# EPFL-IMOS/simple-SFOD

Hardware: AMD Instinct MI355X
Metric: teacher+student train images/s on 1024x2048 synthetic (higher is better)
Workload: dtype bf16x3

## Files before the change

### include/sfod_hip.h

```cpp
#ifndef SFOD_HIP_H
#define SFOD_HIP_H
#include <stdint.h>
#ifdef __cplusplus
extern "C" {
#endif

#define SFOD_F32 0
#define SFOD_BF16 1
#define SFOD_BF16X3 2
#define SFOD_F16X3 3

int sfod_version(void);
const char* sfod_last_error(void);

int sfod_preprocess(const void* const* img_ptrs, const int32_t* sizes, int B, int Hp, int Wp,
                    int Cpad, const float* mean3, const float* std3, void* out, int dt,
                    void* stream);

int sfod_hflip_u8(const void* src, void* dst, int C, int H, int W, void* stream);

int sfod_resize_bilinear_u8(const void* src, void* dst, int C, int H, int W, int h, int w,
                            const int32_t* hbounds, const int32_t* hcoef, int ksize_h,
                            const int32_t* vbounds, const int32_t* vcoef, int ksize_v, int flip,
                            void* stream);

int sfod_conv_fwd(const void* x, const void* w, const float* bias, void* y, int B, int H, int W,
                  int Cin, int Cout, int ksize, int ldy, int act, float* stats, int dt, int out_dt,
                  void* stream);
int sfod_conv_fwd_ws(const void* x, const void* w, const uint32_t* w_absmax, const float* bias, void* y, int B, int H,
                     int W, int Cin, int Cout, int ksize, int ldy, int act, float* stats, int dt, int out_dt,
                     void* stream);
int64_t sfod_conv_fwd_scratch_bytes(int B, int H, int W, int Cin, int Cout, int ksize, int dt, int out_dt, int with_stats);
int sfod_conv_fwd_scratch(const void* x, const void* w, const uint32_t* w_absmax, const float* bias, void* y, int B, int H,
                          int W, int Cin, int Cout, int ksize, int ldy, int act, float* stats, int dt, int out_dt,
                          void* scratch, int64_t scratch_bytes, void* stream);
int sfod_conv_stats_blocks(int B, int H, int W, int Cin, int Cout, int ksize, int dt);
int sfod_set_conv_algo(int algo);
int sfod_conv_dgrad_bnred_blocks(int B, int H, int W, int Cin, int Cout, int dt);
int sfod_conv_dgrad_bnred(const void* x, const void* w, void* dz, int B, int H, int W, int Cin, int Cout, int dt,
                          const float* y, const float* mean, const float* invstd, const float* gamma,
                          const float* beta, float* red_ws, void* stream);
int sfod_conv_fwd_bnin_supported(int B, int H, int W, int Cin, int Cout, int dt);
int sfod_conv_fwd_bnin(const float* x_pre, const float* in_mean, const float* in_invstd, const float* in_gamma,
                       const float* in_beta, const void* w, const float* bias, float* y, int B, int H, int W, int Cin,
                       int Cout, int ldy, int act, float* stats, int dt, void* stream);
int sfod_set_gemm_tile(int tile);
int sfod_set_conv3x3_variant(int variant);
int sfod_last_conv_kernel(char* buf, int n);
int sfod_set_deterministic(int on);
int sfod_get_deterministic(void);
int sfod_set_conv3x3_m16(int on);
int sfod_set_wgrad3x3_pipe(int on);
int sfod_conv_fwd_algo(int B, int H, int W, int Cin, int Cout, int ksize, int dt);

int sfod_conv_first_supported(int B, int H, int W, int Cin, int Cout, int dt, int ldy);
int sfod_conv_first_fused(const void* x, const void* w, const float* bias, const float* scale,
                          const float* shift, void* y, float* stats, int B, int H, int W, int ldy,
                          int act, int dt, void* stream);
int sfod_conv_first_fused_ws(const void* x, const void* w, const uint32_t* w_absmax, const float* bias,
                             const float* scale, const float* shift, void* y, float* stats, int B, int H, int W,
                             int ldy, int act, int dt, void* stream);

int64_t sfod_conv_wgrad_ws_bytes(int B, int H, int W, int Cin, int Cout, int ksize, int lddy, int dt);
int sfod_conv_wgrad(const void* x, const void* dy, float* dw, int B, int H, int W, int Cin,
                    int Cout, int ksize, int lddy, int dt, void* ws, int64_t ws_bytes, void* stream);
int sfod_conv_wgrad_oihw_supported(int B, int H, int W, int Cin, int Cout, int ksize, int lddy, int dt);
int sfod_conv_wgrad_oihw(const void* x, const void* dy, float* dw_oihw, int B, int H, int W, int Cin,
                         int Cout, int ksize, int lddy, int dt, int accumulate, void* ws,
                         int64_t ws_bytes, void* stream);

int sfod_pack_conv_weight(const float* w_oihw, void* w_packed, int Cout, int Cin, int ksize,
                          int CinPad, int rot180, int dt, void* stream);
int sfod_pack_conv_weight_ws(const float* w_oihw, void* w_packed, uint32_t* absmax, int Cout, int Cin, int ksize,
                             int CinPad, int rot180, int dt, void* stream);
int sfod_pack_conv_weights_blocks(int Cout, int Cin, int ksize, int innerPad, int rot180);
int sfod_pack_conv_weights_multi(const int64_t* desc, int n, int total_blocks, int dt, void* stream);
int sfod_pack_conv_weights_multi_ws(const int64_t* desc, int n, int total_blocks, int dt, uint32_t* absmax ,
                                    void* stream);
int sfod_unpack_conv_wgrad(const float* dw_packed, float* dw_oihw, int Cout, int Cin, int ksize,
                           int CinPad, int accumulate, void* stream);
int sfod_pack_fc_weight(const float* w, void* out, int N, int K, int chw_c, int transpose, int dt,
                        void* stream);
int sfod_unpack_fc_wgrad(const float* dw_packed, float* dw, int N, int K, int chw_c,
                         int accumulate, void* stream);
int sfod_pack_fc_weight_ld(const float* w, void* out, int N, int K, int chw_c, int transpose, int ld,
                           int dt, void* stream);
int sfod_pack_fc_weight_ld_ws(const float* w, void* out, uint32_t* absmax, int N, int K, int chw_c, int transpose,
                              int ld, int dt, void* stream);
int sfod_unpack_fc_wgrad_ld(const float* dw_packed, float* dw, int N, int K, int chw_c, int ld,
                            int accumulate, void* stream);
int sfod_bias_grad(const void* dy, float* db, int M, int N, int ld, int accumulate, int dt,
                   void* stream);

int sfod_bn_finalize(const float* stats, int nblocks, int M, int C,
                     float* mean, float* invstd, float* running_mean, float* running_var,
                     float momentum, float eps, int update_running, int64_t* num_batches_tracked,
                     float* ws, void* stream);
int sfod_set_bn_finalize_fused(int on);
int sfod_bn_finalize_ws_floats(int C);
int sfod_bn_relu_pool_fwd(const void* y, const float* mean, const float* invstd,
                          const float* gamma, const float* beta, void* z, int B, int H, int W,
                          int C, int pool, int dt, int out_dt, void* stream);
int sfod_bn_relu_pool_fwd2(const void* y, const float* mean, const float* invstd,
                           const float* gamma, const float* beta, void* z, void* z2, int B, int H, int W,
                           int C, int pool, int dt, int out_dt, void* stream);
int sfod_bn_add_relu_fwd(const void* y, const float* mean, const float* invstd, const float* gamma,
                         const float* beta, const void* residual, void* z, void* z_pairs, void* z_pairs2, int64_t rows,
                         int C, int dt, int pairs_dt, void* stream);
int sfod_bn_relu_pool_bwd(const void* dz, const void* y, const float* mean, const float* invstd,
                          const float* gamma, const float* beta, void* dy, float* dgamma,
                          float* dbeta, float* dgamma_acc, float* dbeta_acc, float* ws, int B, int H,
                          int W, int C, int pool, int dt, int out_dt, int reduced_blocks, void* stream);
#define SFOD_BN_BWD_SCRATCH_ROWS 32
int sfod_bn_bwd_ws_floats(int M, int C);
int sfod_add_act(const void* a, const void* b, void* out, void* out_pairs, void* out_pairs2, int64_t n, int act, int dt,
                 int pairs_dt, void* stream);
int sfod_subsample2(const void* src, void* dst, int B, int H, int W, int C, int backward, int dt,
                    void* stream);
int sfod_stem7x7_supported(int B, int H, int W, int Cp, int dt);
int sfod_stem7x7(const float* x, const void* w_packed, const uint32_t* w_absmax, const float* bias, float* y, int B, int H,
                 int W, int Cp, int act, int dt, void* stream);
int sfod_im2col_stem(const void* x, void* out, int B, int H, int W, int Cp, int Kpad, int dt, int out_dt,
                     void* stream);
int sfod_maxpool3s2(const void* x, void* y, int B, int H, int W, int C, int dt, void* stream);
int sfod_act_bwd(void* dy, const void* y, int64_t n, int act, int dt, void* stream);
int sfod_add_inplace(void* a, const void* b, int64_t n, int dt, void* stream);
int sfod_add_act_bwd(void* a, const void* b, const void* y, int64_t n, int dt, void* stream);
int sfod_mul_mask(void* a, const uint8_t* mask, int64_t n, float scale, int dt, void* stream);

int sfod_rpn_decode(const float* rpn_out, int ld, const float* cell_anchors, int A, int B, int Hf,
                    int Wf, int stride, const int32_t* image_sizes, float* props, float* scores,
                    int32_t* flags, void* stream);
int64_t sfod_sort_ws_bytes(int B, int n);
int sfod_segmented_sort_desc(const float* keys, int B, int n, float* out_keys, int32_t* out_idx,
                             void* ws, int64_t ws_bytes, void* stream);
int sfod_rpn_gather_topk(const float* props, const float* sorted_scores, const int32_t* sorted_idx,
                         int B, int NA, int k, float* cand_boxes, float* cand_scores,
                         uint8_t* cand_valid, void* stream);

int64_t sfod_nms_mask_bytes(int B, int n);
int sfod_nms(const float* boxes, const float* alt_boxes, const int32_t* classes,
             const int32_t* mode, const uint8_t* valid, const int32_t* n_per_image, int B, int n,
             float thr, int max_keep, uint64_t* mask, int32_t* keep_idx, int32_t* keep_count,
             void* stream);
int sfod_gather_kept(const float* cand_boxes, const float* cand_scores, const int32_t* keep_idx,
                     const int32_t* keep_count, int B, int n, int max_keep, float* out_boxes,
                     float* out_scores, void* stream);

int sfod_anchor_match(const float* cell_anchors, int A, int B, int Hf, int Wf, int stride,
                      const float* gt_boxes, const int32_t* gt_count, int Gcap, float lo, float hi,
                      int32_t* matched, int8_t* labels, float* gtmax, void* stream);
int sfod_roi_match(const float* boxes, const int32_t* box_count, int B, int P,
                   const float* gt_boxes, const int32_t* gt_classes, const int32_t* gt_count,
                   int Gcap, float thr, int num_classes, int32_t* matched, int32_t* cls,
                   void* stream);
int sfod_subsample(void* labels_or_cls, const uint32_t* keys, int B, int n, int num, float pos_frac,
                   int bg_label, int mode, int32_t* out_idx, int32_t* out_count, void* stream);

int sfod_rpn_loss(const float* rpn_out, int ld, const float* cell_anchors, int A, int B, int Hf,
                  int Wf, int stride, const int8_t* labels, const int32_t* matched,
                  const float* gt_boxes, const int32_t* gt_count, int Gcap, int batch_per_image,
                  float* loss, const float* grad_scale, float* d_rpn_out, float* ws, void* stream);

int sfod_append_gt(const float* props, const int32_t* prop_count, int B, int P,
                   const float* gt_boxes, const int32_t* gt_count, int Gcap, float* out_boxes,
                   int32_t* out_count, void* stream);
int sfod_roi_build_samples(const float* boxes, const int32_t* cls, const int32_t* matched,
                           const int32_t* samp_idx, const int32_t* samp_count, int B, int P, int S,
                           const float* gt_boxes, const int32_t* gt_count, int Gcap, float* rois,
                           int32_t* gt_cls, float* gt_box, int32_t* n_valid, void* stream);
int sfod_make_rois(const float* props, const int32_t* prop_count, int B, int P, float* rois,
                   void* stream);

int sfod_roi_align_fwd(const void* feat, int B, int H, int W, int C, const float* rois, int R,
                       int pooled, float scale, void* out, int dt, void* stream);
int sfod_roi_align_bwd(const void* dout, int B, int H, int W, int C, const float* rois, int R,
                       int pooled, float scale, float* dfeat, int dt, void* stream);

int sfod_frcnn_loss(const float* pred, int ld, int R, int K, const float* rois,
                    const int32_t* gt_cls, const float* gt_box, const int32_t* n_valid,
                    float* loss, const float* grad_scale, float* d_pred, float* ws, void* stream);

int sfod_frcnn_candidates(const float* pred, int ld, int B, int P, int K, const float* props,
                          const int32_t* prop_count, const int32_t* image_sizes,
                          float score_thresh, float* cand_boxes, float* cand_scores,
                          int32_t* cand_count, void* stream);
int sfod_predict_probs(const float* scores, int ld, int R, int K, float* probs, void* stream);
int sfod_frcnn_prepare_nms(const float* cand_boxes, const float* sorted_scores,
                           const int32_t* sorted_idx, const int32_t* cand_count, int B, int n,
                           int K, int numel_limit, float* s_boxes, float* s_alt_boxes,
                           int32_t* s_classes, int32_t* mode, float* maxcoord_ws, void* stream);
int sfod_frcnn_finalize(const float* s_boxes, const float* sorted_scores, const int32_t* s_classes,
                        const int32_t* keep_idx, const int32_t* keep_count, int B, int n,
                        int max_det, float pseudo_thr, float* det_boxes, float* det_scores,
                        int32_t* det_classes, int32_t* det_count, float* gt_boxes,
                        int32_t* gt_classes, int32_t* gt_count, void* stream);

int sfod_bpc_loss(const float* pred, int ld, int R, int K, const float* rois, const int32_t* roi_cls,
                  int B, const int32_t* image_sizes, const float* gt_boxes, const int32_t* gt_classes,
                  const int32_t* gt_count, int G, float iou_thresh, float* loss, void* ws, void* stream);

int sfod_adaptive_pseudo_labels(const float* det_boxes, const float* det_scores,
                                const int32_t* det_classes, const int32_t* det_count, int B,
                                int max_det, int K, float thr, float* reserve, int R, int row,
                                float* class_acc, int select, float* gt_boxes, int32_t* gt_classes,
// ... 28 lines not shown
```

### simple-sfod_amd/csrc/gemm_conv.hip

```cpp
#include "conv_internal.h"
#include <algorithm>
#include <atomic>

typedef __attribute__((ext_vector_type(8))) __bf16 bf16x8;
typedef __attribute__((ext_vector_type(4))) short s16x4;
typedef __attribute__((ext_vector_type(8))) short s16x8;
typedef __attribute__((ext_vector_type(16))) float f32x16;
typedef __attribute__((ext_vector_type(4))) float f32x4;

#define LDS_PTR(p) ((__attribute__((address_space(3))) void*)(p))
#define GLB_PTR(p) ((const __attribute__((address_space(1))) void*)(p))

__device__ __attribute__((aligned(16))) unsigned int g_zero_page[64];

struct ConvArgs {
  int M;
  int H, W;
  int Cin;
  int Cout;
  int ks;
  int cpt_shift;
  int kchunks;
  int ldy;
  int act;
  const unsigned* wamax;
  int kt_per;
  int nsplit;
  int64_t slab;
};

template <typename T> struct Chunk { static constexpr int E = 16 / sizeof(T); };

__device__ __forceinline__ void glds16(const void* g, void* l) {
  __builtin_amdgcn_global_load_lds(GLB_PTR(g), LDS_PTR(l), 16, 0, 0);
}

__device__ __forceinline__ void chunk_to_tap(int gq, int ks, int cpt_shift, int& tap, int& cc) {
  if (ks == 1) { tap = 0; cc = gq; }
  else { tap = gq >> cpt_shift; cc = gq & ((1 << cpt_shift) - 1); }
}

__device__ __forceinline__ float apply_act(float v, int act) {
  const float slope = (act == 2) ? 0.2f : 1.f;
  return fmaxf(v, (act == 1) ? 0.f : v * slope);
}

template <typename T, typename OutT, int WM, int WN, bool UT, int WR, int NST, int SPLIT = 0, int BKB = 128>
__global__ void __launch_bounds__(WR * 128)
k_conv_fwd(const T* __restrict__ x, const T* __restrict__ w, const float* __restrict__ bias,
           OutT* __restrict__ y, float* __restrict__ stats, ConvArgs a, int tiles_n, int ntiles) {
  static_assert(WM == 2, "wave tile is 64 rows");
  constexpr int NT = WR * 128;
  constexpr int BM = WR * 32 * WM, BN = 64 * WN;
  constexpr int E = Chunk<T>::E;
  constexpr int CPR = BKB / 16;
  constexpr int RPI = 1024 / BKB;
  constexpr int STAGE = (BM + BN) * BKB;
  static_assert(BKB == 128 || BKB == 64, "LDS rows of 128 or 64 bytes");
  extern __shared__ __attribute__((aligned(16))) unsigned char smem[];
  auto swz = [](int r) { return BKB == 128 ? ((r >> 1) & 7) : ((r >> 2) & 3); };

  int bid = blockIdx.x;
  {
    const int q = ntiles / 8, r = ntiles % 8, xcd = bid % 8;
    bid = (xcd < r ? xcd * (q + 1) : r * (q + 1) + (xcd - r) * q) + bid / 8;
  }
  const int tile_n = bid % tiles_n, tile_m = bid / tiles_n;
  const int m0 = tile_m * BM, n0 = tile_n * BN;
  const int lane = threadIdx.x & 63, wave = threadIdx.x >> 6;
  const int wr = wave >> 1, wc = wave & 1;
  const int taps = a.ks * a.ks;
  const int HW = a.H * a.W;

  constexpr int AI = BM / (RPI * 2 * WR), BI = BN / (RPI * 2 * WR);
  static_assert(BI >= 1, "tile too narrow for this wave count");
  int a_row[AI];
  int a_oy[AI], a_ox[AI];
  int64_t a_pix[AI];
  for (int i = 0; i < AI; ++i) {
    const int q = wave * AI + i;
    const int row = q * RPI + lane / CPR;
    a_row[i] = row;
    const int m = m0 + row;
    if (m < a.M) {
      const int rem = m % HW;
      a_oy[i] = rem / a.W;
      a_ox[i] = rem % a.W;
      a_pix[i] = m;
    } else { a_pix[i] = -1; a_oy[i] = 0; a_ox[i] = 0; }
  }
  int b_row[BI];
  for (int i = 0; i < BI; ++i) b_row[i] = (wave * BI + i) * RPI + lane / CPR;
  const int pc = lane % CPR;
  const int KT_all = (a.kchunks + CPR - 1) / CPR;
  const int kt0 = a.kt_per ? (int)blockIdx.y * a.kt_per : 0;
  const int KT = a.kt_per ? min(a.kt_per, KT_all - kt0) : KT_all;
  if (a.kt_per) y += (int64_t)blockIdx.y * a.slab;
  const int64_t wrow_elems = (int64_t)a.kchunks * E;

  int64_t a_base[AI];
  int a_lcs[AI];
  unsigned a_mask[AI];
  int64_t b_base[BI];
  int b_lcs[BI];
  bool b_ok[BI];
  if (UT) {
    for (int i = 0; i < AI; ++i) {
      const int lc = pc ^ swz(a_row[i]);
      a_lcs[i] = lc;
      a_base[i] = (a_pix[i] >= 0 ? a_pix[i] : 0) * a.Cin + (int64_t)lc * E;
      unsigned m = 0;
      if (a_pix[i] >= 0) {
        if (a.ks == 1) m = 1u;
        else
          for (int t = 0; t < 9; ++t) {
            const int iy = a_oy[i] + t / 3 - 1, ix = a_ox[i] + t % 3 - 1;
            if (iy >= 0 && iy < a.H && ix >= 0 && ix < a.W) m |= (1u << t);
          }
      }
      a_mask[i] = m;
    }
    for (int i = 0; i < BI; ++i) {
      const int lc = pc ^ swz(b_row[i]);
      b_lcs[i] = lc;
      const int n = n0 + b_row[i];
      b_ok[i] = n < a.Cout;
      b_base[i] = (int64_t)(b_ok[i] ? n : 0) * wrow_elems + (int64_t)lc * E;
    }
  }

  auto stage_load = [&](int kt, int buf) {
    unsigned char* sA = smem + buf * STAGE;
    unsigned char* sB = sA + BM * BKB;
    kt += kt0;
    if (UT) {
      const int gq0 = kt * CPR;
      int tap = 0, cc0 = gq0;
      if (a.ks != 1) { tap = gq0 >> a.cpt_shift; cc0 = gq0 & ((1 << a.cpt_shift) - 1); }
      const int ky = tap / 3, kx = tap - ky * 3;
      const int64_t delta = (a.ks == 1) ? (int64_t)cc0 * E
                                        : ((int64_t)(ky - 1) * a.W + (kx - 1)) * a.Cin + (int64_t)cc0 * E;
#pragma unroll
      for (int i = 0; i < AI; ++i) {
        const bool ok = ((a_mask[i] >> tap) & 1u) && (gq0 + a_lcs[i] < a.kchunks);
        const void* src = ok ? (const void*)(x + a_base[i] + delta) : (const void*)g_zero_page;
        glds16(src, sA + (wave * AI + i) * 1024);
      }
#pragma unroll
      for (int i = 0; i < BI; ++i) {
        const bool ok = b_ok[i] && (gq0 + b_lcs[i] < a.kchunks);
        const void* src = ok ? (const void*)(w + b_base[i] + (int64_t)gq0 * E) : (const void*)g_zero_page;
        glds16(src, sB + (wave * BI + i) * 1024);
      }
      return;
    }
// ... 909 lines not shown
    bid = (xcd < r ? xcd * (q + 1) : r * (q + 1) + (xcd - r) * q) + bid / 8;
  }
  const int tiles = a.tiles_n * a.tiles_m;
  const int split = bid / tiles, trem = bid % tiles;
  const int n0 = (trem / a.tiles_m) * BN, co0 = (trem % a.tiles_m) * BM;
  const int p_begin = split * a.pix_per_split;
  const int p_end = min(a.M, p_begin + a.pix_per_split);
  if (p_begin >= p_end) return;
  const int taps = a.ks * a.ks;

  int a_prow[AI], a_goff[AI];
  bool a_ok[AI];
  for (int i = 0; i < AI; ++i) {
    const int o = (wave * AI + i) * 1024 + lane * 16;
    const int prow = o / RA, pcol = (o % RA) >> 4;
    const int lc = pcol ^ ((prow & 3) << 2);
    const int col = co0 + (lc & 15) * 8;
    a_prow[i] = prow;
    a_goff[i] = col * 2 + (lc >> 4) * 8;
    a_ok[i] = (col + 8 <= a.lddy) && (col < a.Cout);
  }
  int b_prow[BI], b_tap[BI], b_cc[BI], b_oy[BI], b_ox[BI];
  bool b_ok[BI];
  for (int i = 0; i < BI; ++i) {
    const int o = (wave * BI + i) * 1024 + lane * 16;
    const int prow = o / RB, pcol = (o % RB) >> 4;
    const int lc = pcol ^ ((prow & 3) << 2);
    const int nq = n0 / 8 + (lc & 31);
    int tap, cc;
    chunk_to_tap(nq, a.ks, a.cpt_shift, tap, cc);
    b_prow[i] = prow;
    b_tap[i] = tap;
    b_cc[i] = cc * 2 + (lc >> 5);
    b_ok[i] = (nq < a.nchunks) && (tap < taps);
    const int rem = (p_begin + prow) % (a.H * a.W);
    b_oy[i] = rem / a.W;
    b_ox[i] = rem % a.W;
  }

  auto stage_load = [&](int kt, int buf) {
    unsigned char* sA = smem + buf * STAGE;
    unsigned char* sB = sA + TA;
    const int pbase = p_begin + kt * BKP;
#pragma unroll
    for (int i = 0; i < AI; ++i) {
      const int pix = pbase + a_prow[i];
      const void* src = (pix < p_end && a_ok[i]) ? (const void*)(dy + (int64_t)pix * a.lddy * 2 + a_goff[i])
                                                 : (const void*)g_zero_page;
      glds16(src, sA + (wave * AI + i) * 1024);
    }
#pragma unroll
    for (int i = 0; i < BI; ++i) {
      const int pix = pbase + b_prow[i];
      const void* src = g_zero_page;
      if (pix < p_end && b_ok[i]) {
        if (a.ks == 1) {
          src = x + (int64_t)pix * a.Cin * 2 + (int64_t)b_cc[i] * 8;
        } else {
          const int ky = b_tap[i] / 3, kx = b_tap[i] - ky * 3;
          const int iy = b_oy[i] + ky - 1, ix = b_ox[i] + kx - 1;
          if (iy >= 0 && iy < a.H && ix >= 0 && ix < a.W)
            src = x + ((int64_t)pix + (int64_t)(ky - 1) * a.W + (kx - 1)) * a.Cin * 2 + (int64_t)b_cc[i] * 8;
        }
      }
      glds16(src, sB + (wave * BI + i) * 1024);
      if (a.ks != 1) {
        b_ox[i] += BKP;
        while (b_ox[i] >= a.W) {
          b_ox[i] -= a.W;
          if (++b_oy[i] == a.H) b_oy[i] = 0;
        }
      }
    }
  };

  f32x16 acc[2][2];
  for (int i = 0; i < 2; ++i)
    for (int j = 0; j < 2; ++j)
      for (int r = 0; r < 16; ++r) acc[i][j][r] = 0.f;
  const int h = lane >> 5;
  const int g16 = lane >> 4, t16 = lane & 15;
  const int tq = t16 >> 2, tp = t16 & 3;

  auto stage_compute = [&](int buf) {
    const unsigned char* sA = smem + buf * STAGE;
    const unsigned char* sB = sA + TA;
#pragma unroll
    for (int s = 0; s < BKP / 16; ++s) {
      s16x8 ah[2], al[2], bh[2], bl[2];
#pragma unroll
      for (int e = 0; e < 2; ++e) {
        const int prow = 16 * s + 8 * h + 4 * e + tq;
        const int sw = (prow & 3) << 6;
#pragma unroll
        for (int f = 0; f < 2; ++f) {
          const int ca = (wr * 64 + f * 32 + (g16 & 1) * 16 + 4 * tp) * 2;
          const int cb = (wc * 64 + f * 32 + (g16 & 1) * 16 + 4 * tp) * 2;
          const s16x4 v0 = __builtin_amdgcn_ds_read_tr16_b64_v4i16((__attribute__((address_space(3))) s16x4*)LDS_PTR(sA + prow * RA + (ca ^ sw)));
          const s16x4 v1 = __builtin_amdgcn_ds_read_tr16_b64_v4i16((__attribute__((address_space(3))) s16x4*)LDS_PTR(sA + prow * RA + ((ca + RA / 2) ^ sw)));
          const s16x4 v2 = __builtin_amdgcn_ds_read_tr16_b64_v4i16((__attribute__((address_space(3))) s16x4*)LDS_PTR(sB + prow * RB + (cb ^ sw)));
          const s16x4 v3 = __builtin_amdgcn_ds_read_tr16_b64_v4i16((__attribute__((address_space(3))) s16x4*)LDS_PTR(sB + prow * RB + ((cb + RB / 2) ^ sw)));
#pragma unroll
          for (int k = 0; k < 4; ++k) {
            ah[f][4 * e + k] = v0[k]; al[f][4 * e + k] = v1[k];
            bh[f][4 * e + k] = v2[k]; bl[f][4 * e + k] = v3[k];
          }
        }
      }
#pragma unroll
      for (int i = 0; i < 2; ++i)
#pragma unroll
        for (int j = 0; j < 2; ++j)
          acc[i][j] = __builtin_amdgcn_mfma_f32_32x32x16_bf16(__builtin_bit_cast(bf16x8, ah[i]), __builtin_bit_cast(bf16x8, bl[j]), acc[i][j], 0, 0, 0);
#pragma unroll
      for (int i = 0; i < 2; ++i)
#pragma unroll
        for (int j = 0; j < 2; ++j)
          acc[i][j] = __builtin_amdgcn_mfma_f32_32x32x16_bf16(__builtin_bit_cast(bf16x8, al[i]), __builtin_bit_cast(bf16x8, bh[j]), acc[i][j], 0, 0, 0);
#pragma unroll
      for (int i = 0; i < 2; ++i)
#pragma unroll
        for (int j = 0; j < 2; ++j)
          acc[i][j] = __builtin_amdgcn_mfma_f32_32x32x16_bf16(__builtin_bit_cast(bf16x8, ah[i]), __builtin_bit_cast(bf16x8, bh[j]), acc[i][j], 0, 0, 0);
    }
  };

  const int KT = (p_end - p_begin + BKP - 1) / BKP;
  stage_load(0, 0);
  if (KT > 1) stage_load(1, 1);
  int cur = 0, nxt = 2;
  for (int kt = 0; kt < KT; ++kt) {
    if (kt + 1 < KT) asm volatile("s_waitcnt vmcnt(%0) lgkmcnt(0)" ::"n"(AI + BI) : "memory");
    else asm volatile("s_waitcnt vmcnt(0) lgkmcnt(0)" ::: "memory");
    __builtin_amdgcn_s_barrier();
    asm volatile("" ::: "memory");
    if (kt + 2 < KT) stage_load(kt + 2, nxt);
    stage_compute(cur);
    cur = (cur == 2) ? 0 : cur + 1;
    nxt = (nxt == 2) ? 0 : nxt + 1;
  }
#pragma unroll
  for (int i = 0; i < 2; ++i)
#pragma unroll
    for (int j = 0; j < 2; ++j) {
      const int n = n0 + wc * 64 + j * 32 + (lane & 31);
#pragma unroll
      for (int r = 0; r < 16; ++r) {
        const int co = co0 + wr * 64 + i * 32 + (r & 3) + 8 * (r >> 2) + 4 * h;
        if (co < a.Cout && n < a.Ntot) wg_emit(dw, a, split, co, n, acc[i][j][r]);
      }
    }
}

static bool use_patch_wgrad(const W3Plan& p, int ksize, int dt) {
  if (ksize != 3 || !is_bf16_storage(dt) || dt == SFOD_F16X3 || !p.ok || g_conv_algo == 1) return false;
  if (g_conv_algo == 2) return true;
  return p.nsplit * p.tiles_per_split >= 3;
}

static W3Plan w3_plan_chunked(int B, int H, int W, int Cin, int Cout, int ksize, int lddy, int dt, int& nb) {
  nb = 0;
  W3Plan p;
  p.ok = 0;
  if (ksize != 3 || !is_bf16_storage(dt) || dt == SFOD_F16X3 || (int64_t)B * H * W == 0) return p;
  const int split = (dt == SFOD_BF16X3);
  for (int n = B; n >= 1; n = (n == 1) ? 0 : (n + 1) / 2) {
    p = sfod_w3_plan(n, H, W, Cin, Cout, lddy, split);
    if (p.ok) { nb = n; break; }
  }
  if (!p.ok || !use_patch_wgrad(p, ksize, dt)) { nb = 0; p.ok = 0; }
  return p;
}

static int w3_launch_chunked(const void* x, const void* dy, float* dw, void* ws, int64_t ws_bytes, int B, int H, int W,
                             int Cin, int Cout, int lddy, int dt, int out_mode, int nb, hipStream_t s) {
  const int split = (dt == SFOD_BF16X3);
  const int64_t eb = split ? 4 : 2;
  for (int b0 = 0; b0 < B; b0 += nb) {
    const int n = (B - b0 < nb) ? (B - b0) : nb;
    const W3Plan p = sfod_w3_plan(n, H, W, Cin, Cout, lddy, split);
    if (!p.ok || ws == nullptr || ws_bytes < p.ws_bytes) {
      sfod_set_error("wgrad: workspace too small (sfod_conv_wgrad_ws_bytes)");
      return SFOD_EBADARG;
    }
    const char* xb = (const char*)x + (int64_t)b0 * H * W * Cin * eb;
    const char* dyb = (const char*)dy + (int64_t)b0 * H * W * lddy * eb;
    const int mode = (b0 == 0) ? out_mode : (out_mode == 1 ? 2 : out_mode);
    const int rc = sfod_w3_launch(p, xb, dyb, dw, ws, n, H, W, Cin, Cout, lddy, mode, s, split);
    if (rc) return rc;
  }
  return 0;
}

static std::atomic<int> g_deterministic{-1};
extern "C" int sfod_set_deterministic(int on) {
  g_deterministic.store(on ? 1 : 0, std::memory_order_relaxed);
  return 0;
}
bool sfod_deterministic() {
  int v = g_deterministic.load(std::memory_order_relaxed);
  if (v < 0) {
    const char* ev = getenv("SFOD_DETERMINISTIC");
    int want = (ev && atoi(ev) != 0) ? 1 : 0, expect = -1;
    g_deterministic.compare_exchange_strong(expect, want, std::memory_order_relaxed);
    v = g_deterministic.load(std::memory_order_relaxed);
  }
  return v != 0;
}
extern "C" int sfod_get_deterministic(void) { return sfod_deterministic() ? 1 : 0; }

__global__ void __launch_bounds__(256) k_wgrad_slab_sum(const float* __restrict__ ws, float* __restrict__ dw, int64_t n,
                                                       int nslab, int64_t stride) {
  for (int64_t i = ((int64_t)blockIdx.x * 256 + threadIdx.x) * 4; i < n; i += (int64_t)gridDim.x * 1024) {
    if (i + 4 <= n && (stride & 3) == 0) {
      float4 acc = *reinterpret_cast<const float4*>(dw + i);
      for (int sl = 0; sl < nslab; ++sl) {
        const float4 v = *reinterpret_cast<const float4*>(ws + sl * stride + i);
        acc.x += v.x; acc.y += v.y; acc.z += v.z; acc.w += v.w;
      }
      *reinterpret_cast<float4*>(dw + i) = acc;
    } else {
      for (int64_t e = i; e < n && e < i + 4; ++e) {
        float acc = dw[e];
        for (int sl = 0; sl < nslab; ++sl) acc += ws[sl * stride + e];
        dw[e] = acc;
      }
    }
  }
}

struct GenWgradPlan { int wide, tiles_n, tiles_m, splits, pps; };
static GenWgradPlan gen_wgrad_plan(int M, int Cout, int Ntot, int dt) {
  GenWgradPlan g;
  const int split = (dt == SFOD_BF16X3);
  g.wide = split && Cout >= 128 && Ntot >= 256 && g_conv_algo != 3 &&
           (g_conv_algo == 4 || (int64_t)((Ntot + 255) / 256) * ((Cout + 127) / 128) >= 256);
  if (g.wide) {
    constexpr int BKP = 32;
    g.tiles_n = (Ntot + 255) / 256; g.tiles_m = (Cout + 127) / 128;
    const int tiles = g.tiles_n * g.tiles_m;
    const int max_splits = std::max(1, M / (8 * BKP));
    int best = 1;
    double best_eff = 0.0;
    for (int sp = 1; sp <= std::min(max_splits, 512); ++sp) {
      const int64_t wgs = (int64_t)tiles * sp;
      const double eff = (double)wgs / (double)((wgs + 255) / 256 * 256);
      if (eff > best_eff + 1e-9) { best_eff = eff; best = sp; }
      if (eff >= 0.85 && wgs >= 512) { best = sp; break; }
      if (wgs >= 4096) break;
    }
    int pps = (M + best - 1) / best;
    pps = (pps + BKP - 1) / BKP * BKP;
    g.pps = pps;
    g.splits = (M + pps - 1) / pps;
    return g;
  }
  const int BKP = (dt == SFOD_F32) ? 32 : 64;
  const int TILE = split ? 64 : 128;
  g.tiles_n = (Ntot + TILE - 1) / TILE; g.tiles_m = (Cout + TILE - 1) / TILE;
  int splits = (1024 + g.tiles_n * g.tiles_m - 1) / (g.tiles_n * g.tiles_m);
  const int max_splits = (M + BKP - 1) / BKP;
  if (splits > max_splits) splits = max_splits;
  if (splits < 1) splits = 1;
  int pps = (M + splits - 1) / splits;
  pps = (pps + BKP - 1) / BKP * BKP;
  g.pps = pps;
  g.splits = (M + pps - 1) / pps;
  return g;
}

extern "C" int64_t sfod_conv_wgrad_ws_bytes(int B, int H, int W, int Cin, int Cout, int ksize, int lddy, int dt) {
  if (!(conv_shape_fits(B, H, W, Cin, Cout, ksize) && sfod_ints_ok({lddy}))) return 0;
  int nb = 0;
  if (dt != SFOD_F32) {
    const W3Plan p = w3_plan_chunked(B, H, W, Cin, Cout, ksize, lddy, dt, nb);
    if (nb > 0) return p.ws_bytes;
  }
  if (!sfod_deterministic() || (int64_t)B * H * W == 0) return 0;
  const int Ntot = ksize * ksize * Cin;
  const GenWgradPlan g = gen_wgrad_plan(B * H * W, Cout, Ntot, dt);
  return g.splits > 1 ? (int64_t)g.splits * Cout * Ntot * 4 : 0;
}

extern "C" int sfod_conv_wgrad_oihw_supported(int B, int H, int W, int Cin, int Cout, int ksize, int lddy, int dt) {
  if (!(conv_shape_fits(B, H, W, Cin, Cout, ksize) && sfod_ints_ok({lddy}))) return 0;
  int nb;
  w3_plan_chunked(B, H, W, Cin, Cout, ksize, lddy, dt, nb);
  return nb > 0 ? 1 : 0;
}

extern "C" int sfod_conv_wgrad_oihw(const void* x, const void* dy, float* dw_oihw, int B, int H, int W, int Cin,
                                    int Cout, int ksize, int lddy, int dt, int accumulate, void* ws,
                                    int64_t ws_bytes, void* stream) {
  sfod_note_conv_kernel(nullptr);
  SFOD_REQUIRE(conv_shape_fits(B, H, W, Cin, Cout, ksize) && sfod_ints_ok({lddy}) && sfod_i64s_ok({ws_bytes}),
               "conv_wgrad_oihw: negative or oversized extent");
  SFOD_REQUIRE(x != nullptr && dy != nullptr && dw_oihw != nullptr, "conv_wgrad_oihw: null operand");
  SFOD_REQUIRE(lddy >= Cout, "conv_wgrad_oihw: lddy < Cout");
  int nb;
  w3_plan_chunked(B, H, W, Cin, Cout, ksize, lddy, dt, nb);
  SFOD_REQUIRE(nb > 0, "wgrad_oihw: shape not served by the halo-patch kernel (query sfod_conv_wgrad_oihw_supported)");
  return w3_launch_chunked(x, dy, dw_oihw, ws, ws_bytes, B, H, W, Cin, Cout, lddy, dt, accumulate ? 2 : 1, nb,
                           (hipStream_t)stream);
}

extern "C" int sfod_conv_wgrad(const void* x, const void* dy, float* dw, int B, int H, int W, int Cin,
                               int Cout, int ksize, int lddy, int dt, void* ws, int64_t ws_bytes,
                               void* stream) {
  sfod_note_conv_kernel(nullptr);
  SFOD_REQUIRE(conv_shape_fits(B, H, W, Cin, Cout, ksize) && sfod_ints_ok({lddy}) && sfod_i64s_ok({ws_bytes}),
               "conv_wgrad: negative or oversized extent");
  SFOD_REQUIRE(x != nullptr && dy != nullptr && dw != nullptr, "conv_wgrad: null operand");
  SFOD_REQUIRE(lddy >= Cout, "conv_wgrad: lddy < Cout");
  SFOD_REQUIRE(ksize == 1 || ksize == 3, "wgrad: ksize must be 1 or 3");
  SFOD_REQUIRE(dt == SFOD_F32 || dt == SFOD_BF16 || dt == SFOD_BF16X3, "wgrad: unknown dt");
  const int E = (dt == SFOD_F32) ? 4 : 8;
  SFOD_REQUIRE(Cin % E == 0 && lddy % E == 0, "wgrad: Cin / lddy must be multiples of the 16-byte chunk (bf16x3: of 8)");
  if ((int64_t)B * H * W == 0) return 0;
  const int split = (dt == SFOD_BF16X3);
  SFOD_REQUIRE(!split || Cout % 8 == 0, "wgrad: bf16x3 needs Cout % 8 == 0");
  {
    int nb;
    w3_plan_chunked(B, H, W, Cin, Cout, ksize, lddy, dt, nb);
    if (nb > 0) return w3_launch_chunked(x, dy, dw, ws, ws_bytes, B, H, W, Cin, Cout, lddy, dt, 0, nb, (hipStream_t)stream);
  }
  hipStream_t s = (hipStream_t)stream;
  float* dw_out = dw;
  WgradArgs a;
  a.M = B * H * W; a.H = H; a.W = W; a.Cin = Cin; a.Cout = Cout; a.ks = ksize; a.lddy = lddy;
  const int cpt = Cin / E;
  a.cpt_shift = 0;
  if (ksize == 3) {
    a.cpt_shift = ilog2_exact(cpt);
    SFOD_REQUIRE(a.cpt_shift >= 0, "wgrad3x3: Cin/chunk must be a power of two");
  }
  a.nchunks = ksize * ksize * cpt;
  a.Ntot = ksize * ksize * Cin;
  if (a.M == 0) return 0;
  const GenWgradPlan g = gen_wgrad_plan(a.M, Cout, a.Ntot, dt);
  a.pix_per_split = g.pps;
  a.tiles_n = g.tiles_n;
  a.tiles_m = g.tiles_m;
  a.slab_stride = 0;
  const bool slabs = sfod_deterministic() && g.splits > 1;
  if (slabs) {
    const int64_t need = (int64_t)g.splits * Cout * a.Ntot * 4;
    if (ws == nullptr || ws_bytes < need) {
      sfod_set_error("wgrad: deterministic mode needs the workspace of sfod_conv_wgrad_ws_bytes");
      return SFOD_EBADARG;
    }
    a.slab_stride = (int64_t)Cout * a.Ntot;
    dw_out = (float*)ws;
  }
  const int tiles = g.tiles_n * g.tiles_m;
  if (g.wide) {
    constexpr int LDS = 3 * 32 * (128 + 256) * 4;
    static const hipError_t attr_rc = hipFuncSetAttribute(reinterpret_cast<const void*>(k_conv_wgrad_x3w),
                                                          hipFuncAttributeMaxDynamicSharedMemorySize, LDS);
    SFOD_REQUIRE(attr_rc == hipSuccess, "wgrad: cannot raise the dynamic LDS limit");
    sfod_note_conv_kernel("k_conv_wgrad_x3w");
    hipLaunchKernelGGL(k_conv_wgrad_x3w, dim3(tiles * g.splits), dim3(512), LDS, s, (const bf16_t*)x, (const bf16_t*)dy,
                       dw_out, a);
  } else {
    dim3 grid(tiles * g.splits);
    sfod_note_conv_kernel(dt == SFOD_F32 ? "k_conv_wgrad<float,2,2,0>"
                                         : (split ? "k_conv_wgrad<bf16_t,2,2,1>" : "k_conv_wgrad<bf16_t,2,2,0>"));
    if (dt == SFOD_F32)
      hipLaunchKernelGGL((k_conv_wgrad<float, 2, 2>), grid, dim3(256), 2 * 2 * 32 * 512, s, (const float*)x,
                         (const float*)dy, dw_out, a);
    else if (split)
      hipLaunchKernelGGL((k_conv_wgrad<bf16_t, 2, 2, true>), grid, dim3(256), 2 * 2 * 64 * 256, s, (const bf16_t*)x,
                         (const bf16_t*)dy, dw_out, a);
    else
      hipLaunchKernelGGL((k_conv_wgrad<bf16_t, 2, 2>), grid, dim3(256), 2 * 2 * 64 * 256, s, (const bf16_t*)x,
                         (const bf16_t*)dy, dw_out, a);
  }
  int rc = sfod_check_launch(g.wide ? "conv_wgrad_x3w" : "conv_wgrad");
  if (rc == 0 && slabs) {
    const int64_t n = (int64_t)Cout * a.Ntot;
    hipLaunchKernelGGL(k_wgrad_slab_sum, dim3(cdiv(n, 1024) > 4096 ? 4096 : cdiv(n, 1024)), dim3(256), 0, s,
                       (const float*)ws, dw, n, g.splits, a.slab_stride);
    rc = sfod_check_launch("wgrad_slab_sum");
  }
  return rc;
}
```

### simple-sfod_amd/native.py

```python
import ctypes
import os
import re
import warnings

import torch

warnings.filterwarnings("ignore", message="ComplexHalf support is experimental")

_HERE = os.path.dirname(os.path.abspath(__file__))
HEADER = os.path.join(os.path.dirname(_HERE), "include", "sfod_hip.h")
SO_PATH = os.environ.get("SFOD_HIP_LIB", os.path.join(_HERE, "lib", "libsfod_hip.so"))

F32, BF16, BF16X3, F16X3 = 0, 1, 2, 3

SPLIT_DTYPE = torch.complex32
SPLITH_DTYPE = torch.uint32
PAIR_DTYPES = (SPLIT_DTYPE, SPLITH_DTYPE)

COMPUTE_MODES = {"fp32": F32, "bf16": BF16, "bf16x3": BF16X3, "f16x3": F16X3}


def mode_dt(name):
    try:
        return COMPUTE_MODES[str(name).lower()]
# ... 62 lines not shown
            "(hipcc --offload-arch=gfx950).  There is no CPU fallback for the hot path.")
    lib = ctypes.CDLL(path)
    protos = parse_header()
    for name, (restype, argtypes) in protos.items():
        try:
            fn = getattr(lib, name)
        except AttributeError as e:
            raise NativeLibraryError(f"{path} does not export {name} declared in {HEADER}") from e
        fn.restype = restype
        fn.argtypes = argtypes
    _lib, _protos = lib, protos
    return lib


def exported_symbols():
    load()
    return sorted(_protos)


def _chk(rc, name):
    if rc != 0:
        msg = _lib.sfod_last_error().decode()
        raise NativeLibraryError(f"{name} failed with code {rc}: {msg}")


_raw_stream = getattr(torch._C, "_cuda_getCurrentRawStream", None)


def _stream():
    if _raw_stream is not None:
        return _raw_stream(torch.cuda.current_device())
    return torch.cuda.current_stream().cuda_stream


def _p(t):
    if t is None:
        return None
    assert t.is_cuda, "native ops need device tensors"
    assert t.is_contiguous(), "native ops need contiguous tensors"
    return t.data_ptr()


def dt_of(t):
    if t.dtype == torch.float32:
        return F32
    if t.dtype == torch.bfloat16:
        return BF16
    if t.dtype == SPLIT_DTYPE:
        return BF16X3
    if t.dtype == SPLITH_DTYPE:
        return F16X3
    raise TypeError(f"unsupported dtype {t.dtype}")


def dt_of_dtype(dtype):
    return {torch.float32: F32, torch.bfloat16: BF16, SPLIT_DTYPE: BF16X3, SPLITH_DTYPE: F16X3}[dtype]


def torch_dtype(dt):
    return {F32: torch.float32, BF16: torch.bfloat16, BF16X3: SPLIT_DTYPE, F16X3: SPLITH_DTYPE}[dt]


def chunk_elems(dt):
    return 4 if dt == F32 else 8


def nhwc_operand(x_nchw, dtype):
    p = x_nchw.permute(0, 2, 3, 1)
    if p.dtype == dtype:
        return p.contiguous()
    if dtype in PAIR_DTYPES or p.dtype in PAIR_DTYPES:
        return cast(p.contiguous(), dtype)
    return p.to(dtype).contiguous()


def as_operand(t, dtype):
    return t if t.dtype == dtype else cast(t, dtype)


def operands_for(t, dtype, need_grad):
    gdt = grad_dtype_of(dtype)
    if not need_grad:
        return as_operand(t, dtype), None
    if gdt == dtype:
        op = as_operand(t, dtype)
        return op, op
    if t.dtype == torch.float32 and dtype == SPLITH_DTYPE and gdt == SPLIT_DTYPE:
        t = t.contiguous()
        a = torch.empty(t.shape, dtype=SPLITH_DTYPE, device=t.device)
        b = torch.empty(t.shape, dtype=SPLIT_DTYPE, device=t.device)
        call("sfod_cast_pairs_both", t, a, b, t.numel())
        return a, b
    return as_operand(t, dtype), as_operand(t, gdt)


class _Everything:
    def __contains__(self, item):
        return True


class KernelTimer:

    def __init__(self, watch=("sfod_conv_fwd", "sfod_conv_wgrad", "sfod_conv_wgrad_oihw")):
        self.watch = _Everything() if watch is None else set(watch)
        self.records = []

    def summary(self):
        torch.cuda.synchronize()
        out = {}
        for name, flops, a, b in self.records:
            d = out.setdefault(name, {"launches": 0, "ms": 0.0, "flops": 0.0})
            d["launches"] += 1
            d["ms"] += a.elapsed_time(b)
            d["flops"] += flops
        return out


_timer = None
_pending_flops = 0.0
_pending_tag = ""


def set_timer(timer):
    global _timer
    _timer = timer


def call(name, *args, timer_name=None):
    global _pending_flops
    lib = load()
    conv = [(_p(a) if isinstance(a, torch.Tensor) else a) for a in args]
    if _timer is not None and (timer_name or name) in _timer.watch:
        a, b = torch.cuda.Event(enable_timing=True), torch.cuda.Event(enable_timing=True)
        a.record()
        rc = getattr(lib, name)(*conv, _stream())
        b.record()
        _timer.records.append(((timer_name or name) + _pending_tag, _pending_flops, a, b))
        _pending_flops = 0.0
    else:
        rc = getattr(lib, name)(*conv, _stream())
    _chk(rc, name)


def query(name, *args):
    return getattr(load(), name)(*args)


def set_conv_algo(algo):
    load().sfod_set_conv_algo(int(algo))


def set_wgrad3x3_pipe(on):
    load().sfod_set_wgrad3x3_pipe(int(on))


def set_gemm_tile(tile):
    load().sfod_set_gemm_tile(int(tile))


def set_conv3x3_variant(variant):
    load().sfod_set_conv3x3_variant(int(variant))


def last_conv_kernel():
    buf = ctypes.create_string_buffer(256)
    n = load().sfod_last_conv_kernel(buf, len(buf))
    if n < 0:
        _chk(n, "sfod_last_conv_kernel")
    return buf.value.decode()


def set_deterministic(on):
    lib = load()
    prev = bool(lib.sfod_get_deterministic())
    lib.sfod_set_deterministic(int(bool(on)))
    return prev


def set_bn_finalize_fused(on):
    load().sfod_set_bn_finalize_fused(int(bool(on)))


def set_conv3x3_m16(on):
    load().sfod_set_conv3x3_m16(int(on))


_const_cache = {}


def dev_const(values, dtype, device):
    key = (values, dtype, str(device))
    t = _const_cache.get(key)
    if t is None:
        if len(_const_cache) > 4096:
            _const_cache.clear()
        t = torch.tensor(values, dtype=dtype).to(device)
        _const_cache[key] = t
    return t


_PIN_SLOTS, _PIN_WIDTH = 32, 64
_pin_ring = {}


def _pinned_upload_i64(values, dev):
    n = len(values)
    if n > _PIN_WIDTH:
        return torch.tensor(values, dtype=torch.int64).to(dev)
    st = _pin_ring.get(dev)
    if st is None:
        st = {"buf": torch.empty(_PIN_SLOTS, _PIN_WIDTH, dtype=torch.int64).pin_memory(), "ev": [None] * _PIN_SLOTS,
              "next": 0}
        _pin_ring[dev] = st
    i = st["next"]
    st["next"] = (i + 1) % _PIN_SLOTS
    if st["ev"][i] is not None:
        st["ev"][i].synchronize()
    slot = st["buf"][i, :n]
    slot.copy_(torch.tensor(values, dtype=torch.int64))
    out = slot.to(dev, non_blocking=True)
    ev = torch.cuda.Event()
    ev.record()
    st["ev"][i] = ev
    return out


def preprocess(images_u8, Hp, Wp, cpad, mean, std, dt):
    dev = images_u8[0].device
    B = len(images_u8)
    imgs = [im.contiguous() for im in images_u8]
    ptrs = _pinned_upload_i64([im.data_ptr() for im in imgs], dev)
    sizes = dev_const(tuple((int(im.shape[1]), int(im.shape[2])) for im in imgs), torch.int32, dev)
    out = torch.empty(B, Hp, Wp, cpad, dtype=torch_dtype(dt), device=dev)
    m = (ctypes.c_float * 3)(*mean)
    s = (ctypes.c_float * 3)(*std)
    lib = load()
    rc = lib.sfod_preprocess(ptrs.data_ptr(), sizes.data_ptr(), B, Hp, Wp, cpad,
                             ctypes.cast(m, ctypes.c_void_p), ctypes.cast(s, ctypes.c_void_p),
                             out.data_ptr(), dt, _stream())
    _chk(rc, "sfod_preprocess")
    out._keepalive = (imgs, ptrs)
    return out, sizes


def pil_bilinear_coeffs(in_size, out_size):
    import math
    import numpy as np
    scale = float(in_size) / float(out_size)
    filterscale = scale if scale >= 1.0 else 1.0
    support = 1.0 * filterscale
    ksize = int(math.ceil(support)) * 2 + 1
    bounds = np.zeros((out_size, 2), dtype=np.int32)
    kk = np.zeros((out_size, ksize), dtype=np.int32)
    ss = 1.0 / filterscale
    for xx in range(out_size):
        center = (xx + 0.5) * scale
        xmin = int(center - support + 0.5)
        if xmin < 0:
            xmin = 0
        xmax = int(center + support + 0.5)
        if xmax > in_size:
            xmax = in_size
        xmax -= xmin
        k = [0.0] * ksize
        ww = 0.0
        for x in range(xmax):
            a = abs((x + xmin - center + 0.5) * ss)
            w = 1.0 - a if a < 1.0 else 0.0
            k[x] = w
            ww += w
        for x in range(xmax):
            if ww != 0.0:
                k[x] /= ww
        bounds[xx] = (xmin, xmax)
        for x in range(ksize):
            v = k[x] * (1 << 22)
            kk[xx, x] = int(v - 0.5) if k[x] < 0 else int(v + 0.5)
    return bounds, kk, ksize


_resize_tabs = {}


def resize_bilinear_u8(img, newh, neww, flip=False):
    assert img.dtype == torch.uint8 and img.dim() == 3
    img = img.contiguous()
    C, H, W = img.shape
    key = (img.device, H, W, newh, neww)
    tabs = _resize_tabs.get(key)
    if tabs is None:
        hb, hk, ksh = pil_bilinear_coeffs(W, neww)
        vb, vk, ksv = pil_bilinear_coeffs(H, newh)
        tabs = tuple(torch.from_numpy(a).to(img.device) for a in (hb, hk, vb, vk)) + (ksh, ksv)
        _resize_tabs[key] = tabs
    hb, hk, vb, vk, ksh, ksv = tabs
    out = torch.empty(C, newh, neww, dtype=torch.uint8, device=img.device)
    call("sfod_resize_bilinear_u8", img, out, C, H, W, newh, neww, hb, hk, ksh, vb, vk, ksv, int(flip))
    return out


AUG_BRIGHTNESS, AUG_CONTRAST, AUG_SATURATION, AUG_HUE, AUG_GRAYSCALE = 0, 1, 2, 3, 4
_aug_ws = {}


def aug_color(img, ops):
    assert img.dtype == torch.uint8 and img.dim() == 3 and img.shape[0] == 3
# ... 746 lines not shown
```

Before: 158.7.

## Add six-stage ring-buffered wide wgrad kernel with transposed LDS reads

Adds a new bf16x3 weight-gradient kernel that streams dy and x through a six-deep LDS ring using direct global-to-LDS loads. It reads MFMA fragments with ds_read_b64_tr_b16 transposed reads and remaps block ids by XCD. When the tile count is large it skips the split-K search and accumulates directly into dw, avoiding atomics and slab reductions. It is on by default (env or setter can disable) and adds knobs to force the split count. The risks are lower occupancy from the larger LDS footprint and less parallelism when splits are dropped.

```diff
diff --git a/include/sfod_hip.h b/include/sfod_hip.h
--- a/include/sfod_hip.h
+++ b/include/sfod_hip.h
@@ -51,6 +51,9 @@
 int sfod_get_deterministic(void);
 int sfod_set_conv3x3_m16(int on);
 int sfod_set_wgrad3x3_pipe(int on);
+int sfod_set_wgrad_wide(int mode);
+int sfod_get_wgrad_wide(void);
+int sfod_set_wgrad_splits(int n);
 int sfod_conv_fwd_algo(int B, int H, int W, int Cin, int Cout, int ksize, int dt);
 
 int sfod_conv_first_supported(int B, int H, int W, int Cin, int Cout, int dt, int ldy);
diff --git a/simple-sfod_amd/csrc/gemm_conv.hip b/simple-sfod_amd/csrc/gemm_conv.hip
--- a/simple-sfod_amd/csrc/gemm_conv.hip
+++ b/simple-sfod_amd/csrc/gemm_conv.hip
@@ -1,6 +1,7 @@
 #include "conv_internal.h"
 #include <algorithm>
 #include <atomic>
+#include <climits>
 
 typedef __attribute__((ext_vector_type(8))) __bf16 bf16x8;
 typedef __attribute__((ext_vector_type(4))) short s16x4;
@@ -1216,6 +1217,197 @@
     }
 }
 
+template <int N> __device__ __forceinline__ void wgr_wait_vm() {
+  asm volatile("s_waitcnt vmcnt(%0)" ::"n"(N) : "memory");
+}
+__device__ __forceinline__ void wgr_wait_lds() {
+  asm volatile("s_waitcnt lgkmcnt(0)" ::: "memory");
+  __builtin_amdgcn_sched_barrier(0);
+}
+template <int OFF> __device__ __forceinline__ s16x4 wgr_tr_read(unsigned addr) {
+  s16x4 v;
+  asm volatile("ds_read_b64_tr_b16 %0, %1 offset:%2" : "=v"(v) : "v"(addr), "n"(OFF));
+  return v;
+}
+__device__ __forceinline__ bf16x8 wgr_cat8(s16x4 a, s16x4 b) {
+  return __builtin_bit_cast(bf16x8, __builtin_shufflevector(a, b, 0, 1, 2, 3, 4, 5, 6, 7));
+}
+
+template <bool KS1>
+__global__ void __launch_bounds__(512)
+k_conv_wgrad_x3r(const bf16_t* __restrict__ x, const bf16_t* __restrict__ dy, float* __restrict__ dw, WgradArgs a) {
+  constexpr int BM = 128, BN = 256, BKP = 16, NBUF = 6;
+  constexpr int RA = BM * 4, RB = BN * 4;
+  constexpr int TA = BKP * RA, TB = BKP * RB, STEP = TA + TB;
+  constexpr int BI = TB / 1024 / 8;
+  static_assert(TA == 8 * 1024 && BI == 2, "one dy and two x DMA instructions per wave and k-step");
+  extern __shared__ __attribute__((aligned(16))) unsigned char smem[];
+  const int lane = threadIdx.x & 63, wave = threadIdx.x >> 6;
+  const int wr = wave >> 2, wc = wave & 3;
+  int bid = blockIdx.x;
+  {
+    const int nt = gridDim.x, q = nt / 8, r = nt % 8, xcd = bid % 8;
+    bid = (xcd < r ? xcd * (q + 1) : r * (q + 1) + (xcd - r) * q) + bid / 8;
+  }
+  const int tiles = a.tiles_n * a.tiles_m;
+  const int split = bid / tiles, trem = bid % tiles;
+  const int n0 = (trem / a.tiles_m) * BN, co0 = (trem % a.tiles_m) * BM;
+  const int p_begin = split * a.pix_per_split;
+  const int p_end = min(a.M, p_begin + a.pix_per_split);
+  if (p_begin >= p_end) return;
+
+  const bf16_t* a_src;
+  int a_pix, a_lim;
+  {
+    const int o = wave * 1024 + lane * 16;
+    const int prow = o / RA, pcol = (o % RA) >> 4;
+    const int lc = pcol ^ ((prow & 3) << 2);
+    const int col = co0 + (lc & 15) * 8;
+    a_pix = p_begin + prow;
+    a_lim = ((col + 8 <= a.lddy) && (col < a.Cout)) ? p_end : INT_MIN;
+    a_src = dy + (int64_t)a_pix * a.lddy * 2 + (col * 2 + (lc >> 4) * 8);
+  }
+  const int64_t a_adv = (int64_t)BKP * a.lddy * 2;
+  const bf16_t* b_src[BI];
+  int b_pix[BI], b_lim[BI];
+  int b_ky[BI], b_kx[BI], b_oy[BI], b_ox[BI];
+  for (int i = 0; i < BI; ++i) {
+    const int o = (wave * BI + i) * 1024 + lane * 16;
+    const int prow = o / RB, pcol = (o % RB) >> 4;
+    const int lc = pcol ^ ((prow & 3) << 2);
+    const int nq = n0 / 8 + (lc & 31);
+    int tap, cc;
+    chunk_to_tap(nq, KS1 ? 1 : a.ks, a.cpt_shift, tap, cc);
+    b_pix[i] = p_begin + prow;
+    b_lim[i] = ((nq < a.nchunks) && (tap < (KS1 ? 1 : a.ks * a.ks))) ? p_end : INT_MIN;
+    b_ky[i] = KS1 ? 1 : tap / 3;
+    b_kx[i] = KS1 ? 1 : tap - (tap / 3) * 3;
+    const int rem = KS1 ? 0 : b_pix[i] % (a.H * a.W);
+    b_oy[i] = KS1 ? 0 : rem / a.W;
+    b_ox[i] = KS1 ? 0 : rem % a.W;
+    b_src[i] = x + ((int64_t)b_pix[i] + (int64_t)(b_ky[i] - 1) * a.W + (b_kx[i] - 1)) * a.Cin * 2 +
+               (int64_t)(cc * 2 + (lc >> 5)) * 8;
+  }
+  const int64_t b_adv = (int64_t)BKP * a.Cin * 2;
+
+  auto dma_step = [&](int buf) {
+    unsigned char* sA = smem + buf * STEP;
+    unsigned char* sB = sA + TA;
+    glds16((a_pix < a_lim) ? (const void*)a_src : (const void*)g_zero_page, sA + wave * 1024);
+    a_pix += BKP;
+    a_src += a_adv;
+#pragma unroll
+    for (int i = 0; i < BI; ++i) {
+      bool ok = b_pix[i] < b_lim[i];
+      if constexpr (!KS1) {
+        const int iy = b_oy[i] + b_ky[i] - 1, ix = b_ox[i] + b_kx[i] - 1;
+        ok = ok && iy >= 0 && iy < a.H && ix >= 0 && ix < a.W;
+        b_ox[i] += BKP;
+        while (b_ox[i] >= a.W) {
+          b_ox[i] -= a.W;
+          if (++b_oy[i] == a.H) b_oy[i] = 0;
+        }
+      }
+      glds16(ok ? (const void*)b_src[i] : (const void*)g_zero_page, sB + (wave * BI + i) * 1024);
+      b_pix[i] += BKP;
+      b_src[i] += b_adv;
+    }
+  };
+
+  const int h = lane >> 5;
+  const int g16 = lane >> 4, t16 = lane & 15;
+  const int tq = t16 >> 2, tp = t16 & 3;
+  unsigned fa[2], fb[2];
+#pragma unroll
+  for (int f = 0; f < 2; ++f) {
+    const int ca = (wr * 64 + f * 32 + (g16 & 1) * 16 + 4 * tp) * 2;
+    const int cb = (wc * 64 + f * 32 + (g16 & 1) * 16 + 4 * tp) * 2;
+    fa[f] = (unsigned)((8 * h + tq) * RA + (ca ^ (tq << 6)));
+    fb[f] = (unsigned)(TA + (8 * h + tq) * RB + (cb ^ (tq << 6)));
+  }
+  const unsigned lds0 = (unsigned)(uintptr_t)LDS_PTR(smem);
+  s16x4 ra[8], rb[8];
+  auto read_step = [&](int buf) {
+    const unsigned base = lds0 + (unsigned)(buf * STEP);
+#pragma unroll
+    for (int f = 0; f < 2; ++f) {
+      const unsigned pa = base + fa[f], pb = base + fb[f];
+      ra[4 * f + 0] = wgr_tr_read<0>(pa);               ra[4 * f + 1] = wgr_tr_read<RA / 2>(pa);
+      ra[4 * f + 2] = wgr_tr_read<4 * RA>(pa);          ra[4 * f + 3] = wgr_tr_read<4 * RA + RA / 2>(pa);
+      rb[4 * f + 0] = wgr_tr_read<0>(pb);               rb[4 * f + 1] = wgr_tr_read<RB / 2>(pb);
+      rb[4 * f + 2] = wgr_tr_read<4 * RB>(pb);          rb[4 * f + 3] = wgr_tr_read<4 * RB + RB / 2>(pb);
+    }
+  };
+  bf16x8 ah[2], al[2], bh[2], bl[2];
+  auto take_frags = [&]() {
+#pragma unroll
+    for (int f = 0; f < 2; ++f) {
+      ah[f] = wgr_cat8(ra[4 * f + 0], ra[4 * f + 2]); al[f] = wgr_cat8(ra[4 * f + 1], ra[4 * f + 3]);
+      bh[f] = wgr_cat8(rb[4 * f + 0], rb[4 * f + 2]); bl[f] = wgr_cat8(rb[4 * f + 1], rb[4 * f + 3]);
+    }
+  };
+
+  f32x16 acc[2][2];
+  for (int i = 0; i < 2; ++i)
+    for (int j = 0; j < 2; ++j)
+      for (int r = 0; r < 16; ++r) acc[i][j][r] = 0.f;
+
+  const int KT = (p_end - p_begin + BKP - 1) / BKP;
+  for (int s = 0; s < NBUF; ++s) dma_step(s);
+  wgr_wait_vm<(NBUF - 1) * 3>();
+  __builtin_amdgcn_s_barrier();
+  asm volatile("" ::: "memory");
+  read_step(0);
+  wgr_wait_lds();
+  take_frags();
+  int cur = 0;
+  for (int kt = 0; kt < KT; ++kt) {
+    const int nxt = (cur == NBUF - 1) ? 0 : cur + 1;
+    wgr_wait_vm<(NBUF - 2) * 3>();
+    __builtin_amdgcn_s_barrier();
+    asm volatile("" ::: "memory");
+    dma_step(cur);
+    __builtin_amdgcn_sched_barrier(0);
+#pragma unroll
+    for (int i = 0; i < 2; ++i)
+#pragma unroll
+      for (int j = 0; j < 2; ++j)
+        acc[i][j] = __builtin_amdgcn_mfma_f32_32x32x16_bf16(ah[i], bl[j], acc[i][j], 0, 0, 0);
+    __builtin_amdgcn_sched_barrier(0);
+    read_step(nxt);
+    __builtin_amdgcn_sched_barrier(0);
+#pragma unroll
+    for (int i = 0; i < 2; ++i)
+#pragma unroll
+      for (int j = 0; j < 2; ++j)
+        acc[i][j] = __builtin_amdgcn_mfma_f32_32x32x16_bf16(al[i], bh[j], acc[i][j], 0, 0, 0);
+#pragma unroll
+    for (int i = 0; i < 2; ++i)
+#pragma unroll
+      for (int j = 0; j < 2; ++j)
+        acc[i][j] = __builtin_amdgcn_mfma_f32_32x32x16_bf16(ah[i], bh[j], acc[i][j], 0, 0, 0);
+    __builtin_amdgcn_sched_barrier(0);
+    wgr_wait_lds();
+    take_frags();
+    cur = nxt;
+  }
+  wgr_wait_vm<0>();
+#pragma unroll
+  for (int i = 0; i < 2; ++i)
+#pragma unroll
+    for (int j = 0; j < 2; ++j) {
+      const int n = n0 + wc * 64 + j * 32 + (lane & 31);
+#pragma unroll
+      for (int r = 0; r < 16; ++r) {
+        const int co = co0 + wr * 64 + i * 32 + (r & 3) + 8 * (r >> 2) + 4 * h;
+        if (co < a.Cout && n < a.Ntot) {
+          if (a.slab_stride < 0) dw[(int64_t)co * a.Ntot + n] += acc[i][j][r];
+          else wg_emit(dw, a, split, co, n, acc[i][j][r]);
+        }
+      }
+    }
+}
+
 static bool use_patch_wgrad(const W3Plan& p, int ksize, int dt) {
   if (ksize != 3 || !is_bf16_storage(dt) || dt == SFOD_F16X3 || !p.ok || g_conv_algo == 1) return false;
   if (g_conv_algo == 2) return true;
@@ -1291,6 +1483,30 @@
       }
     }
   }
+}
+
+static std::atomic<int> g_wgrad_wide{-1};
+extern "C" int sfod_set_wgrad_wide(int mode) {
+  SFOD_REQUIRE(mode == 0 || mode == 1, "set_wgrad_wide: mode must be 0 or 1");
+  g_wgrad_wide.store(mode, std::memory_order_relaxed);
+  return 0;
+}
+static int wgrad_wide_mode() {
+  int v = g_wgrad_wide.load(std::memory_order_relaxed);
+  if (v < 0) {
+    const char* ev = getenv("SFOD_WGRAD_WIDE");
+    int want = (ev && atoi(ev) == 0) ? 0 : 1, expect = -1;
+    g_wgrad_wide.compare_exchange_strong(expect, want, std::memory_order_relaxed);
+    v = g_wgrad_wide.load(std::memory_order_relaxed);
+  }
+  return v;
+}
+extern "C" int sfod_get_wgrad_wide(void) { return wgrad_wide_mode(); }
+static std::atomic<int> g_wgrad_splits{0};
+extern "C" int sfod_set_wgrad_splits(int n) {
+  SFOD_REQUIRE(n >= 0 && n <= 512, "set_wgrad_splits: 0 .. 512");
+  g_wgrad_splits.store(n, std::memory_order_relaxed);
+  return 0;
 }
 
 struct GenWgradPlan { int wide, tiles_n, tiles_m, splits, pps; };
@@ -1306,7 +1522,10 @@
     const int max_splits = std::max(1, M / (8 * BKP));
     int best = 1;
     double best_eff = 0.0;
-    for (int sp = 1; sp <= std::min(max_splits, 512); ++sp) {
+    const int forced = g_wgrad_splits.load(std::memory_order_relaxed);
+    const bool unsplit = wgrad_wide_mode() == 1 && tiles >= 2 * 256;
+    if (forced > 0) best = std::min(forced, std::max(1, M / BKP));
+    for (int sp = 1; forced == 0 && !unsplit && sp <= std::min(max_splits, 512); ++sp) {
       const int64_t wgs = (int64_t)tiles * sp;
       const double eff = (double)wgs / (double)((wgs + 255) / 256 * 256);
       if (eff > best_eff + 1e-9) { best_eff = eff; best = sp; }
@@ -1406,6 +1625,8 @@
   a.tiles_n = g.tiles_n;
   a.tiles_m = g.tiles_m;
   a.slab_stride = 0;
+  const bool ring = g.wide && wgrad_wide_mode() == 1;
+  if (ring && g.splits == 1) a.slab_stride = -1;
   const bool slabs = sfod_deterministic() && g.splits > 1;
   if (slabs) {
     const int64_t need = (int64_t)g.splits * Cout * a.Ntot * 4;
@@ -1417,7 +1638,21 @@
     dw_out = (float*)ws;
   }
   const int tiles = g.tiles_n * g.tiles_m;
-  if (g.wide) {
+  if (ring) {
+    constexpr int LDS = 6 * 16 * (128 + 256) * 4;
+    static const hipError_t attr_rc1 = hipFuncSetAttribute(reinterpret_cast<const void*>(k_conv_wgrad_x3r<true>),
+                                                           hipFuncAttributeMaxDynamicSharedMemorySize, LDS);
+    static const hipError_t attr_rc3 = hipFuncSetAttribute(reinterpret_cast<const void*>(k_conv_wgrad_x3r<false>),
+                                                           hipFuncAttributeMaxDynamicSharedMemorySize, LDS);
+    SFOD_REQUIRE(attr_rc1 == hipSuccess && attr_rc3 == hipSuccess, "wgrad: cannot raise the dynamic LDS limit");
+    sfod_note_conv_kernel(ksize == 1 ? "k_conv_wgrad_x3r<1x1>" : "k_conv_wgrad_x3r<taps>");
+    if (ksize == 1)
+      hipLaunchKernelGGL(k_conv_wgrad_x3r<true>, dim3(tiles * g.splits), dim3(512), LDS, s, (const bf16_t*)x,
+                         (const bf16_t*)dy, dw_out, a);
+    else
+      hipLaunchKernelGGL(k_conv_wgrad_x3r<false>, dim3(tiles * g.splits), dim3(512), LDS, s, (const bf16_t*)x,
+                         (const bf16_t*)dy, dw_out, a);
+  } else if (g.wide) {
     constexpr int LDS = 3 * 32 * (128 + 256) * 4;
     static const hipError_t attr_rc = hipFuncSetAttribute(reinterpret_cast<const void*>(k_conv_wgrad_x3w),
                                                           hipFuncAttributeMaxDynamicSharedMemorySize, LDS);
diff --git a/simple-sfod_amd/native.py b/simple-sfod_amd/native.py
--- a/simple-sfod_amd/native.py
+++ b/simple-sfod_amd/native.py
@@ -238,6 +238,17 @@
 
 def set_wgrad3x3_pipe(on):
     load().sfod_set_wgrad3x3_pipe(int(on))
+
+
+def set_wgrad_wide(mode):
+    lib = load()
+    prev = int(lib.sfod_get_wgrad_wide())
+    _chk(lib.sfod_set_wgrad_wide(int(mode)), "sfod_set_wgrad_wide")
+    return prev
+
+
+def set_wgrad_splits(n):
+    _chk(load().sfod_set_wgrad_splits(int(n)), "sfod_set_wgrad_splits")
 
 
 def set_gemm_tile(tile):
```

Measured after the change: 159.5, median of 6. Within noise of the previous version (+0.5%).
